# emsig/emg3d

Measured on AMD Instinct MI355X. Metric: Mcells*smoother-iters/s (fp64) per multigrid cycle, higher is better.
Workload: dtype c128 (complex fp64)

## Files before the change

emg3d_amd/_cycle.py:

```python
import os

import numpy as np
import torch

from emg3d_amd import _lib

__all__ = ['run_cycles', 'coarse_correction', 'coarse_schedule', 'smooth_level', 'stop_reason',
           'ConvergenceError', 'current_sc_dir', 'current_lr_dir']


class ConvergenceError(Exception):
    """Multigrid as preconditioner diverged or stagnated: aborts the Krylov solver."""


def current_sc_dir(sc_dir, grid):
    kept = tuple(n % 2 != 0 or n < 3 or sc_dir == axis + 1 for axis, n in enumerate(grid.shape_cells))
    codes = {(0, 0, 0): 0, (1, 0, 0): 1, (0, 1, 0): 2, (0, 0, 1): 3, (0, 1, 1): 4, (1, 0, 1): 5, (1, 1, 0): 6,
             (1, 1, 1): 6}
    return codes[tuple(int(k) for k in kept)]


_LR_AXES = {0: (), 1: (1,), 2: (2,), 3: (3,), 4: (2, 3), 5: (1, 3), 6: (1, 2), 7: (1, 2, 3)}
_LR_CODE = {axes: code for code, axes in _LR_AXES.items()}


def current_lr_dir(lr_dir, grid):
    axes = tuple(a for a in _LR_AXES[int(lr_dir)] if grid.shape_cells[a - 1] != 2)
    return _LR_CODE[axes]


def smooth_level(lv, nu, lr_dir, var):
    axes = _LR_AXES[current_lr_dir(lr_dir, lv.grid)]
# ... 28 lines not shown
            stack.pop()
            continue
        if level == depth:
            steps.append((SMOOTH, level, nu_coarse, "coarsest level", done, visits))
            frame[2] = done + 1
            continue
        if nu_pre > 0:
            steps.append((SMOOTH, level, nu_pre, "pre-smoothing", done, visits))
        steps.append((DOWN, level, 0))
        frame[3] = True
        steps.append((ENTER, level + 1, 0))
        stack.append([level + 1, _visits(cycle, cycmax, depth, level + 1, visits - done), 0, False])
    return steps


def _visits(cycle, cycmax, depth, level, budget):
    if level == depth:
        return 1
    if budget == 0 or cycle != 'F':
        return cycmax
    return budget


class CoarseCorrection:

    def __init__(self, first, first_level, var):
        self.var = var
        self.levels = {first_level: first}

    def run(self, steps):
        var = self.var
        loud = var.verb > 4
        trace = var.first_cycle and var.verb > 3
        sc_at = {}
        for step in steps:
            kind, level = step[0], step[1]
            lv = self.levels[level]
            if kind == SMOOTH:
                smooth_level(lv, step[2], var.lr_dir, var)
                if loud:
                    _log_smoothing(var, level, lv, step[3], step[4], step[5])
            elif kind == DOWN:
                sc_at[level] = current_sc_dir(var.sc_dir, lv.grid)
                lv.residual(store=True, norm=False)
                self.levels[level + 1] = lv.restrict_to(sc_at[level])
            elif kind == UP:
                lv.prolong_from(sc_at[level])
                if trace:
                    var.level_all.append(level)
            elif trace:
                var.level_all.append(level)


def _log_smoothing(var, level, lv, what, it=0, cycmax=None):
    n = lv.grid.shape_cells
    norm = lv.residual(store=False, norm=True)
    visits = var.cycmax if cycmax is None else cycmax
    var.cprint(f"     {it:2} {level} {visits} [{n[0]:3}, {n[1]:3}, {n[2]:3}]: {norm:.3e} {what}", 4)


USE_GRAPHS = os.environ.get('EMG3D_AMD_GRAPHS', '1') != '0'
GRAPH_AFTER = int(os.environ.get('EMG3D_AMD_GRAPH_AFTER', '2'))
CONCURRENT = 0


def coarse_correction(clv, var, budget, first_level=1, graphed=None, top=None):
    depth = int(var.clevel[var.sc_dir])
    steps = coarse_schedule(var.cycle, var.cycmax, depth, first_level, budget, var.nu_pre, var.nu_coarse,
                            var.nu_post)
    clv.work.factor_epoch += 1
    runner = CoarseCorrection(clv, first_level, var)
    if graphed is None:
        graphed = first_level == 1 and var.verb < 5 and USE_GRAPHS and CONCURRENT == 0
    if not graphed:
        runner.run(steps)
        return
    cache = clv.__dict__.setdefault('_graphs', {})
    key = (int(var.sc_dir), int(var.lr_dir), budget, var.cycle, var.nu_pre, var.nu_post, var.nu_coarse, depth,
           float(getattr(var, 'smoother_omega', 1.0)), _lib.options_fingerprint())
    entry = cache.get(key)
    if entry is None or entry['graph'] is None:
        if entry is None:
            stale = [k for k in cache if k[-1] != key[-1]]
            if stale:
                for k in stale:
                    del cache[k]
                root = top if top is not None else clv
                _purge_stale_graphs(root, key[-1])
                _drop_stale_point_factors(root)
            entry = cache[key] = {'work': None, 'graph': None, 'seen': 0}
        if entry['seen'] < GRAPH_AFTER:
            before = var.smoother_cell_sweeps
            runner.run(steps)
            entry['work'] = var.smoother_cell_sweeps - before
            entry['seen'] += 1
            return
        before = var.smoother_cell_sweeps
        torch.cuda.synchronize()
        graph = torch.cuda.CUDAGraph()
        with torch.cuda.graph(graph, capture_error_mode='thread_local'):
            runner.run(steps)
        entry['work'] = var.smoother_cell_sweeps - before
        var.smoother_cell_sweeps = before
        entry['graph'] = graph
    entry['graph'].replay()
    var.smoother_cell_sweeps += entry['work']


def _purge_stale_graphs(lv, fingerprint, seen=None):
    seen = set() if seen is None else seen
    if id(lv) in seen:
        return
    seen.add(id(lv))
    cache = lv.__dict__.get('_graphs')
    if cache:
        for k in [k for k in cache if k[-1] != fingerprint]:
            del cache[k]
    for link in lv.children.values():
        _purge_stale_graphs(link['level'], fingerprint, seen)


def _drop_stale_point_factors(lv, seen=None):
    seen = set() if seen is None else seen
    if id(lv) in seen:
        return
    seen.add(id(lv))
    now = ('point', _lib.lib().emg3d_get_option(b'point_tile_min'))
    for k in [k for k in lv._factors if isinstance(k, tuple) and k[0] == 'point' and k != now]:
        del lv._factors[k]
    for link in lv.children.values():
        _drop_stale_point_factors(link['level'], seen)


def stop_reason(var, l2_last, l2_stag, it):
# ... 173 lines not shown
```

emg3d_amd/_device.py:

```python
import ctypes

import numpy as np
import torch

from emg3d_amd import _lib, meshes
from emg3d_amd import core as _core

_vp = ctypes.c_void_p


def _stream():
    return _vp(torch.cuda.current_stream().cuda_stream)


def _ptr(t, offset_elems=0):
    return _vp(t.data_ptr() + offset_elems * t.element_size())


def coarsen_flags(sc_dir):
    return (sc_dir not in (1, 5, 6), sc_dir not in (2, 4, 6), sc_dir not in (3, 4, 5))


def interp_table(cnodes, nodes):
    i = np.searchsorted(cnodes, nodes) - 1
# ... 381 lines not shown
                ccc = (cgrid.cell_centers_x, cgrid.cell_centers_y, cgrid.cell_centers_z)[d]
                for w in _core.restrict_weights(nodes, cc, g.h[d], cnodes, ccc, cgrid.h[d]):
                    slots.append(len(fparts))
                    fparts.append(np.ascontiguousarray(w, dtype=np.float64))
            else:
                slots += [None, None, None]
        tabs = [interp_table(cn, n) for cn, n in ((cgrid.nodes_x, g.nodes_x),
                                                  (cgrid.nodes_y, g.nodes_y),
                                                  (cgrid.nodes_z, g.nodes_z))]
        pw_slots = []
        for t in tabs:
            pw_slots.append(len(fparts))
            fparts.append(t[1])
        foff = np.cumsum([0] + [a.size for a in fparts])
        fbuf = self.work.upload(np.concatenate(fparts))
        ioff = np.cumsum([0] + [t[0].size for t in tabs])
        ibuf = self.work.upload(np.concatenate([t[0] for t in tabs]))
        wptr = [(_ptr(fbuf, int(foff[i])) if i is not None else None) for i in slots]
        pwptr = [_ptr(fbuf, int(foff[i])) for i in pw_slots]
        ilptr = [_ptr(ibuf, int(ioff[d])) for d in range(3)]
        link = {'level': clevel, 'buffers': (fbuf, ibuf), 'wptr': wptr, 'ilptr': ilptr, 'pwptr': pwptr}
        self.children[sc_dir] = link
        return link

    def restrict_to(self, sc_dir):
        link = self.child(sc_dir)
        c = link['level']
        nx, ny, nz = self.grid.shape_cells
        _lib.check(_lib.lib().emg3d_dev_restrict_clear_batch(
            *c.parts(c.s), *c.parts(c.e), *self.parts(self.r), *link['wptr'], nx, ny, nz, sc_dir,
            self.is_complex, self.batch, self.grid.n_edges, c.grid.n_edges, _stream()), 'emg3d_dev_restrict')
        return c

    def prolong_from(self, sc_dir):
        link = self.children[sc_dir]
        c = link['level']
        nx, ny, nz = self.grid.shape_cells
        _lib.check(_lib.lib().emg3d_dev_prolong_batch(
            *self.parts(self.e), *c.parts(c.e), *link['ilptr'], *link['pwptr'], nx, ny, nz, sc_dir,
            self.is_complex, self.batch, self.grid.n_edges, c.grid.n_edges, _stream()),
            'emg3d_dev_prolong')
```

emg3d_amd/_lib.py:

```python
import ctypes
import os
import subprocess

_HERE = os.path.dirname(os.path.abspath(__file__))
CSRC = os.path.join(_HERE, 'csrc')
LIBDIR = os.path.join(_HERE, 'lib')
LIBPATH = os.path.join(LIBDIR, 'libemg3d_amd.so')
HEADER = os.path.join(os.path.dirname(_HERE), 'include', 'emg3d_amd.h')
SOURCES = [os.path.join(CSRC, f) for f in ('kernels.hip', 'stencil.h', 'launch.h', 'cplx.h', 'receivers.h', 'krylov.h',
                                            'adjoint.h', 'reciprocal.h', 'hessian.h', 'gram.h')] + [HEADER]

HIPCC_FLAGS = ['--offload-arch=gfx950', '-O3', '-std=c++17', '-fPIC', '-shared', '-ffp-contract=fast-honor-pragmas']


class Emg3dAmdError(RuntimeError):
    """A C-ABI call returned a non-zero status."""


def build(force=False, verbose=False):
    os.makedirs(LIBDIR, exist_ok=True)
    stale = (not os.path.exists(LIBPATH) or
             any(os.path.getmtime(s) > os.path.getmtime(LIBPATH) for s in SOURCES))
    if force or stale:
        hipcc = os.environ.get('HIPCC', 'hipcc')
# ... 21 lines not shown
    'emg3d_version': (_ci, []),
    'emg3d_last_error': (ctypes.c_char_p, []),
    'emg3d_device_count': (_ci, []),
    'emg3d_set_option': (_ci, [ctypes.c_char_p, _ci]),
    'emg3d_get_option': (_ci, [ctypes.c_char_p]),
    'emg3d_option_count': (_ci, []),
    'emg3d_option_name': (ctypes.c_char_p, [_ci]),
    'emg3d_options_generation': (_ci, []),
    'emg3d_line_kernel_name': (ctypes.c_char_p, [_ci] * 6),
    'emg3d_core_amat_x': (_ci, [_vp] * 13 + [_ci] * 4),
    'emg3d_core_gauss_seidel': (_ci, [_ci] + [_vp] * 13 + [_ci] * 5),
    'emg3d_core_restrict': (_ci, [_vp] * 15 + [_ci] * 5),
    'emg3d_core_blocks_to_amat': (_ci, [_vp] * 5 + [_ci] * 4),
    'emg3d_core_solve': (_ci, [_vp, _vp, _ci, _ci]),
    'emg3d_gs_scratch_bytes': (_sz, [_ci] * 5),
    'emg3d_line_fac_bytes': (_sz, [_ci] * 5),
    'emg3d_line_fac_bytes_lv': (_sz, [ctypes.POINTER(Level), _ci]),
    'emg3d_line_compact_used': (_ci, [ctypes.POINTER(Level), _ci]),
    'emg3d_point_compact_used': (_ci, [ctypes.POINTER(Level)]),
    'emg3d_line_lfac_bytes': (_sz, [_ci] * 4),
    'emg3d_dev_line_setup': (_ci, [ctypes.POINTER(Level), _ci, _vp, _vp, _vp]),
    'emg3d_point_fac_bytes': (_sz, [_ci] * 4),
    'emg3d_point_fac_bytes_lv': (_sz, [ctypes.POINTER(Level)]),
    'emg3d_dev_eta_is_imaginary': (_ci, [ctypes.POINTER(Level), ctypes.POINTER(_ci), _vp]),
    'emg3d_dev_point_setup': (_ci, [ctypes.POINTER(Level), _vp, _vp]),
    'emg3d_dev_gauss_seidel': (_ci, [ctypes.POINTER(Level), _ci, _ci, _vp, _vp, _vp, _sz, _vp]),
    'emg3d_residual_ws_len': (_sz, [_ci] * 3),
    'emg3d_dev_residual': (_ci, [ctypes.POINTER(Level), _vp, _vp, _vp, _vp, _sz, _vp, _vp]),
    'emg3d_dev_restrict': (_ci, [_vp] * 15 + [_ci] * 5 + [_vp]),
    'emg3d_dev_prolong': (_ci, [_vp] * 12 + [_ci] * 5 + [_vp]),
    'emg3d_dev_restrict_batch': (_ci, [_vp] * 15 + [_ci] * 6 + [_sz, _sz, _vp]),
    'emg3d_dev_restrict_clear_batch': (_ci, [_vp] * 18 + [_ci] * 6 + [_sz, _sz, _vp]),
    'emg3d_dev_prolong_batch': (_ci, [_vp] * 12 + [_ci] * 6 + [_sz, _sz, _vp]),
    'emg3d_dev_restrict_param': (_ci, [_vp, _vp] + [_ci] * 5 + [_vp]),
    'emg3d_dev_pec_zero': (_ci, [_vp] * 3 + [_ci] * 4 + [_vp]),
    'emg3d_krylov_ws_len': (_sz, []),
    'emg3d_dev_krylov_step': (_ci, [_sz, _ci, _vp, _ci, _vp, _vp, _vp, _ci, _vp, _vp, _vp, _ci, _vp, _vp, _vp, _sz, _vp]),
    'emg3d_dev_apply_operator': (_ci, [ctypes.POINTER(Level), _vp, _vp, _vp, _vp]),
    'emg3d_dev_zero': (_ci, [_vp, _sz, _vp]),
    'emg3d_dev_copy': (_ci, [_vp, _vp, _sz, _vp]),
    'emg3d_dev_gradient_accumulate': (_ci, [_ci] * 4 + [_vp] * 6 + [ctypes.c_double] * 2 + [_vp] * 5),
    'emg3d_dev_sensitivity_source': (_ci, [_ci] * 4 + [_vp] * 3 + [ctypes.c_double] * 2 + [_vp] * 7 + [_vp]),
    'emg3d_dev_edge_weights': (_ci, [_ci] * 3 + [_vp] * 7 + [_vp]),
    'emg3d_sensitivity_dots_ws_len': (_sz, [_ci, _ci, _sz]),
    'emg3d_dev_sensitivity_dots': (_ci, [_sz, _ci, _vp, _sz, _ci, _vp, _sz, _ci, _vp] + [ctypes.c_double] * 2 +
                                   [_vp, _vp, _sz, _vp]),
    'emg3d_dev_sensitivity_combine': (_ci, [_sz, _ci, _vp, _sz, _ci, _vp, _sz, _ci, _vp, _vp, _vp]),
    'emg3d_dev_edges_to_cells': (_ci, [_ci] * 4 + [_vp] * 3 + [ctypes.c_double] * 2 + [_vp] * 4 + [_vp]),
    'emg3d_dev_hessian_diagonal': (_ci, [_ci] * 4 + [_vp, _sz, _ci, _vp, _sz, _ci, _vp] + [_ci] * 3 + [ctypes.c_double] +
                                   [_vp, _vp, _sz, _vp]),
    'emg3d_data_gram_ws_len': (_sz, [_ci] * 6),
    'emg3d_dev_data_gram': (_ci, [_ci] * 4 + [_vp, _sz, _ci, _vp, _sz, _ci] + [ctypes.c_double] * 2 +
                            [_vp, _sz, _ci, _vp, _sz, _ci] + [ctypes.c_double] * 2 + [_ci] * 3 +
                            [_vp, _sz, _vp, _vp, _sz, _vp, _sz, _vp]),
    'emg3d_dev_source_field': (_ci, [_ci] * 4 + [_vp] * 7 + [_ci] + [ctypes.c_double] * 2 + [_vp] * 4),
    'emg3d_dev_volume_model': (_ci, [_ci] * 4 + [_vp] * 5 + [_ci] + [_vp] * 3 + [ctypes.c_double] * 4 + [_vp] * 5),
    'emg3d_dev_magnetic_field': (_ci, [_ci] * 4 + [_vp] * 7 + [ctypes.c_double] * 2 + [_vp] * 4),
    'emg3d_dev_spline_filter': (_ci, [_vp] + [_ci] * 4 + [_vp]),
    'emg3d_dev_spline_eval': (_ci, [_vp] + [_ci] * 4 + [_vp, _ci, _vp, _vp]),
    'emg3d_dev_linear_eval': (_ci, [_vp] + [_ci] * 4 + [_vp, _vp, _ci, _vp, _vp]),
    'emg3d_dev_volume_average': (_ci, [_vp] + [_ci] * 3 + [_vp] * 10 + [_ci] * 3 + [_vp, _ci, _vp]),
}

LEVEL_ETA_IMAG = 1
LEVEL_LINE_COMPACT = 2
LEVEL_POINT_COMPACT = 4
# ... 45 lines not shown
```

emg3d_amd/csrc/kernels.hip:

```cpp
#include <hip/hip_runtime.h>

#include <algorithm>
#include <climits>
#include <cstdio>
#include <cstdlib>
#include <cstring>
#include <string>
#include <type_traits>

#include "../../include/emg3d_amd.h"
#include "launch.h"

using emg::cplx;

namespace {

thread_local std::string g_err;

int fail(int code, const char *what)
{
    g_err = what;
    return code;
}

// ... 1339 lines not shown
        if (tid == 0) {
            const int bid = blockIdx.x + gridDim.x * (blockIdx.y + gridDim.y * blockIdx.z);
            partial[bid] = (wsum[0] + wsum[1]) + (wsum[2] + wsum[3]);
        }
    }
}

__global__ __launch_bounds__(256) void k_reduce_sum(const double *partial, int n, double *out)
{
    partial += (size_t)blockIdx.x * n;
    out += blockIdx.x;
    __shared__ double sm[256];
    double acc = 0.0;
    for (int i = threadIdx.x; i < n; i += 256) acc += partial[i];
    sm[threadIdx.x] = acc;
    __syncthreads();
    for (int s = 128; s > 0; s >>= 1) {
        if ((int)threadIdx.x < s) sm[threadIdx.x] += sm[threadIdx.x + s];
        __syncthreads();
    }
    if (threadIdx.x == 0) *out = sm[0];
}

template <class T> __global__ __launch_bounds__(256) void k_restrict(emg::Restrict<T> R)
{
    const int cix = blockIdx.x * blockDim.x + threadIdx.x;
    const int ciy = blockIdx.y * blockDim.y + threadIdx.y;
    const int b = blockIdx.z / R.cnzn, ciz = blockIdx.z - b * R.cnzn;
    if (cix >= R.cnxn || ciy >= R.cnyn) return;
    R.rx += b * R.fstride; R.ry += b * R.fstride; R.rz += b * R.fstride;
    R.crx += b * R.cstride; R.cry += b * R.cstride; R.crz += b * R.cstride;
    if (R.cex) { R.cex += b * R.cstride; R.cey += b * R.cstride; R.cez += b * R.cstride; }
    emg::restrict_node<T>(R, cix, ciy, ciz);
}

template <class T> __global__ __launch_bounds__(256) void k_prolong(emg::Prolong<T> P)
{
    const int ix = blockIdx.x * blockDim.x + threadIdx.x;
    const int iy = blockIdx.y * blockDim.y + threadIdx.y;
    const int b = blockIdx.z / (P.nz + 1), iz = blockIdx.z - b * (P.nz + 1);
    if (ix > P.nx || iy > P.ny) return;
    P.ex += b * P.fstride; P.ey += b * P.fstride; P.ez += b * P.fstride;
    P.cex += b * P.cstride; P.cey += b * P.cstride; P.cez += b * P.cstride;
    emg::prolong_cell<T>(P, ix, iy, iz);
}

template <class T>
__global__ __launch_bounds__(256) void k_restrict_param(T *out, const T *in, int nx, int ny, int cnx,
                                                        int cny, int fx, int fy, int fz)
{
    const int cix = blockIdx.x * blockDim.x + threadIdx.x;
    const int ciy = blockIdx.y * blockDim.y + threadIdx.y;
    const int ciz = blockIdx.z;
    if (cix >= cnx || ciy >= cny) return;
    emg::restrict_param_cell<T>(out, in, nx, ny, cnx, cny, fx, fy, fz, cix, ciy, ciz);
}

template <class T>
__global__ __launch_bounds__(256) void k_pec_zero(T *ex, T *ey, T *ez, int nx, int ny, int nz)
{
    const int ix = blockIdx.x * blockDim.x + threadIdx.x;
    const int iy = blockIdx.y * blockDim.y + threadIdx.y;
    const int iz = blockIdx.z;
    if (ix > nx || iy > ny) return;
    const bool bx = ix == 0 || ix == nx, by = iy == 0 || iy == ny, bz = iz == 0 || iz == nz;
    if (ix < nx && (by || bz)) ex[ix + nx * (iy + (ny + 1) * iz)] = emg::zero<T>();
// ... 369 lines not shown
template <class T>
int launch_restrict(void *crx, void *cry, void *crz, const void *rx, const void *ry, const void *rz,
                    const double *const w[9], int nx, int ny, int nz, int sc_dir, hipStream_t st, int batch = 1,
                    size_t fstride = 0, size_t cstride = 0, void *cex = nullptr, void *cey = nullptr, void *cez = nullptr)
{
    const ScDirs f = sc_flags(sc_dir);
    if ((f.cx && nx % 2) || (f.cy && ny % 2) || (f.cz && nz % 2))
        return fail(EMG3D_ERR_BADARG, "restrict: odd cell count in a coarsened direction");
    emg::Restrict<T> R = emg::make_restrict<T>(crx, cry, crz, rx, ry, rz, w, nx, ny, nz, sc_dir);
    R.batch = batch > 1 ? batch : 1; R.fstride = fstride; R.cstride = cstride;
    R.cex = (T *)cex; R.cey = (T *)cey; R.cez = (T *)cez;
    const emg::Dim3 g = emg::cell_grid(R.cnxn, R.cnyn, R.cnzn);
    hipLaunchKernelGGL(k_restrict<T>, dim3(g.x, g.y, g.z * R.batch), d3(emg::cell_block()), 0, st, R);
    HIP_TRY(hipGetLastError());
    return 0;
}

template <class T>
int launch_prolong(void *ex, void *ey, void *ez, const void *cex, const void *cey, const void *cez,
                   const int32_t *ilx, const int32_t *ily, const int32_t *ilz, const double *wx,
                   const double *wy, const double *wz, int nx, int ny, int nz, int sc_dir, hipStream_t st,
                   int batch = 1, size_t fstride = 0, size_t cstride = 0)
{
    emg::Prolong<T> P =
        emg::make_prolong<T>(ex, ey, ez, cex, cey, cez, ilx, ily, ilz, wx, wy, wz, nx, ny, nz, sc_dir);
    P.batch = batch > 1 ? batch : 1; P.fstride = fstride; P.cstride = cstride;
    const emg::Dim3 g = emg::cell_grid(nx + 1, ny + 1, nz + 1);
    hipLaunchKernelGGL(k_prolong<T>, dim3(g.x, g.y, g.z * P.batch), d3(emg::cell_block()), 0, st, P);
    HIP_TRY(hipGetLastError());
    return 0;
}

template <class T>
int launch_restrict_param(void *out, const void *in, int nx, int ny, int nz, int sc_dir, hipStream_t st)
{
    const ScDirs f = sc_flags(sc_dir);
    const int fx = f.cx ? 2 : 1, fy = f.cy ? 2 : 1, fz = f.cz ? 2 : 1;
    const int cnx = nx / fx, cny = ny / fy, cnz = nz / fz;
    const dim3 block = d3(emg::cell_block());
    const dim3 grid = d3(emg::cell_grid(cnx, cny, cnz));
    hipLaunchKernelGGL(k_restrict_param<T>, grid, block, 0, st, (T *)out, (const T *)in, nx, ny, cnx, cny, fx, fy, fz);
    HIP_TRY(hipGetLastError());
    return 0;
}


struct DevBuf {
    void *d = nullptr;
    size_t bytes = 0;
    ~DevBuf() { if (d) (void)hipFree(d); }
    hipError_t up(const void *h, size_t n)
    {
        bytes = n;
        hipError_t e = hipMalloc(&d, n ? n : 1);
        if (e != hipSuccess) return e;
        return n ? hipMemcpy(d, h, n, hipMemcpyHostToDevice) : hipSuccess;
    }
    hipError_t alloc(size_t n)
    {
        bytes = n;
        return hipMalloc(&d, n ? n : 1);
    }
    hipError_t down(void *h) const { return bytes ? hipMemcpy(h, d, bytes, hipMemcpyDeviceToHost) : hipSuccess; }
};

struct Sizes {
// ... 310 lines not shown
    const double *const w[9] = {wxl, wx0, wxr, wyl, wy0, wyr, wzl, wz0, wzr};
    return is_complex ? launch_restrict<cplx>(crx, cry, crz, rx, ry, rz, w, nx, ny, nz, sc_dir, (hipStream_t)stream, batch,
                                              fine_stride, coarse_stride)
                      : launch_restrict<double>(crx, cry, crz, rx, ry, rz, w, nx, ny, nz, sc_dir, (hipStream_t)stream,
                                                batch, fine_stride, coarse_stride);
}

int emg3d_dev_restrict_clear_batch(void *crx, void *cry, void *crz, void *cex, void *cey, void *cez, const void *rx,
                                   const void *ry, const void *rz, const double *wxl, const double *wx0,
                                   const double *wxr, const double *wyl, const double *wy0, const double *wyr,
                                   const double *wzl, const double *wz0, const double *wzr, int nx, int ny, int nz,
                                   int sc_dir, int is_complex, int batch, size_t fine_stride, size_t coarse_stride,
                                   void *stream)
{
    if (sc_dir < 0 || sc_dir > 6) return fail(EMG3D_ERR_BADARG, "restrict: sc_dir must be 0..6");
    if (!cex || !cey || !cez) return fail(EMG3D_ERR_BADARG, "restrict_clear: coarse field missing");
    const double *const w[9] = {wxl, wx0, wxr, wyl, wy0, wyr, wzl, wz0, wzr};
    return is_complex ? launch_restrict<cplx>(crx, cry, crz, rx, ry, rz, w, nx, ny, nz, sc_dir, (hipStream_t)stream, batch,
                                              fine_stride, coarse_stride, cex, cey, cez)
                      : launch_restrict<double>(crx, cry, crz, rx, ry, rz, w, nx, ny, nz, sc_dir, (hipStream_t)stream,
                                                batch, fine_stride, coarse_stride, cex, cey, cez);
}

int emg3d_dev_prolong_batch(void *ex, void *ey, void *ez, const void *cex, const void *cey, const void *cez,
                            const int32_t *ilx, const int32_t *ily, const int32_t *ilz, const double *wx,
                            const double *wy, const double *wz, int nx, int ny, int nz, int sc_dir, int is_complex,
                            int batch, size_t fine_stride, size_t coarse_stride, void *stream)
{
    if (sc_dir < 0 || sc_dir > 6) return fail(EMG3D_ERR_BADARG, "prolong: sc_dir must be 0..6");
    return is_complex ? launch_prolong<cplx>(ex, ey, ez, cex, cey, cez, ilx, ily, ilz, wx, wy, wz, nx, ny, nz, sc_dir,
                                             (hipStream_t)stream, batch, fine_stride, coarse_stride)
                      : launch_prolong<double>(ex, ey, ez, cex, cey, cez, ilx, ily, ilz, wx, wy, wz, nx, ny, nz, sc_dir,
                                               (hipStream_t)stream, batch, fine_stride, coarse_stride);
}

int emg3d_dev_restrict_param(void *out, const void *in, int nx, int ny, int nz, int sc_dir, int is_complex,
                             void *stream)
{
    if (sc_dir < 0 || sc_dir > 6) return fail(EMG3D_ERR_BADARG, "restrict_param: sc_dir must be 0..6");
    return is_complex ? launch_restrict_param<cplx>(out, in, nx, ny, nz, sc_dir, (hipStream_t)stream)
                      : launch_restrict_param<double>(out, in, nx, ny, nz, sc_dir, (hipStream_t)stream);
}

int emg3d_dev_pec_zero(void *ex, void *ey, void *ez, int nx, int ny, int nz, int is_complex, void *stream)
{
    const dim3 block = d3(emg::cell_block());
    const dim3 grid = d3(emg::cell_grid(nx + 1, ny + 1, nz + 1));
    if (is_complex)
        hipLaunchKernelGGL(k_pec_zero<cplx>, grid, block, 0, (hipStream_t)stream, (cplx *)ex, (cplx *)ey, (cplx *)ez, nx, ny, nz);
    else
        hipLaunchKernelGGL(k_pec_zero<double>, grid, block, 0, (hipStream_t)stream, (double *)ex, (double *)ey, (double *)ez, nx, ny, nz);
    HIP_TRY(hipGetLastError());
    return 0;
}


int emg3d_core_amat_x(void *rx, void *ry, void *rz, const void *ex, const void *ey, const void *ez,
                      const void *eta_x, const void *eta_y, const void *eta_z, const double *zeta,
                      const double *hx, const double *hy, const double *hz, int nx, int ny, int nz,
                      int is_complex)
{
    if (emg3d_device_count() < 1) return fail(EMG3D_ERR_NODEVICE, "no HIP device");
    const Sizes S(nx, ny, nz, is_complex);
    DevBuf drx, dry, drz, dex, dey, dez, dz, dhx, dhy, dhz;
    EtaUpload eta;
    HIP_TRY(drx.up(rx, S.nex * S.esz)); HIP_TRY(dry.up(ry, S.ney * S.esz)); HIP_TRY(drz.up(rz, S.nez * S.esz));
// ... 138 lines not shown
```

emg3d_amd/csrc/launch.h:

```cpp
#pragma once
#include "stencil.h"

namespace emg {

struct Dim3 { int x, y, z; };

inline int cdiv(int a, int b) { return (a + b - 1) / b; }
EMG_HD int fast_div(int a, int b) { return (int)(((float)a + 0.5f) / (float)b); }
inline int cnt_par(int n, int par) { return par ? n / 2 : (n - 1) / 2; }
EMG_HD int first_par(int par) { return par ? 1 : 2; }

inline int mirrored_colour(int iback, int cc)
{
    const int seq[4] = {0, 2, 3, 1};
    return seq[iback ? 3 - cc : cc];
}
inline int &point_order_ref() { static int order = 1; return order; }
inline int sweep_colour(int iback, int cc)
{
    return mirrored_colour(point_order_ref() == 0 ? iback : 0, cc);
}
inline int line_sweep_colour(int order, int it, int cc)
{
    if (order == 0) return mirrored_colour((it + 1) & 1, cc);
// ... 486 lines not shown
        for (int r = 0; r < 5; ++r) rhs[r] = zero<T>();
    }
    T *o = vec + ((size_t)k * (cntp * cntq) + lid) * 5;
#pragma unroll
    for (int r = 0; r < 5; ++r) o[r] = rhs[r];
}

template <class T, int DIR>
EMG_HD void line_scatter_thread(const Level<T> &L, int colour, int cntp, int cntq, int tp, int tq, int k,
                                const T *vec)
{
    int i1, i2, lid;
    if (!line_of_thread<DIR>(colour, cntp, cntq, tp, tq, i1, i2, lid)) return;
    const Axes<T, DIR> A(L);
    line_scatter<T, DIR>(A, k, i1, i2, vec + ((size_t)k * (cntp * cntq) + lid) * 5);
}

inline Dim3 linequad_block() { return Dim3{64, 1, 1}; }
inline Dim3 linequad_grid(const LineClass &c) { return Dim3{cdiv(c.lines * 4, 64), 1, 1}; }

inline Dim3 cell_block() { return Dim3{64, 4, 1}; }
inline Dim3 cell_grid(int n1, int n2, int n3) { return Dim3{cdiv(n1, 64), cdiv(n2, 4), n3}; }

struct ScDirs { int cx, cy, cz; };
inline ScDirs sc_flags(int sc_dir)
{
    ScDirs f;
    f.cx = !(sc_dir == 1 || sc_dir == 5 || sc_dir == 6);
    f.cy = !(sc_dir == 2 || sc_dir == 4 || sc_dir == 6);
    f.cz = !(sc_dir == 3 || sc_dir == 4 || sc_dir == 5);
    return f;
}

template <class T>
inline Restrict<T> make_restrict(void *crx, void *cry, void *crz, const void *rx, const void *ry,
                                 const void *rz, const double *const w[9], int nx, int ny, int nz, int sc_dir)
{
    const ScDirs f = sc_flags(sc_dir);
    Restrict<T> R;
    R.cx = f.cx; R.cy = f.cy; R.cz = f.cz;
    R.nxn = nx + 1; R.nyn = ny + 1; R.nzn = nz + 1;
    R.cnxn = (f.cx ? nx / 2 : nx) + 1; R.cnyn = (f.cy ? ny / 2 : ny) + 1; R.cnzn = (f.cz ? nz / 2 : nz) + 1;
    R.rx = (const T *)rx; R.ry = (const T *)ry; R.rz = (const T *)rz;
    R.crx = (T *)crx; R.cry = (T *)cry; R.crz = (T *)crz;
    for (int i = 0; i < 3; ++i) { R.wx[i] = w[i]; R.wy[i] = w[3 + i]; R.wz[i] = w[6 + i]; }
    return R;
}

template <class T>
inline Prolong<T> make_prolong(void *ex, void *ey, void *ez, const void *cex, const void *cey, const void *cez,
                               const int *ilx, const int *ily, const int *ilz, const double *wx,
                               const double *wy, const double *wz, int nx, int ny, int nz, int sc_dir)
{
    const ScDirs f = sc_flags(sc_dir);
    Prolong<T> P;
    P.cx = f.cx; P.cy = f.cy; P.cz = f.cz;
    P.nx = nx; P.ny = ny; P.nz = nz;
    P.cnx = f.cx ? nx / 2 : nx; P.cny = f.cy ? ny / 2 : ny; P.cnz = f.cz ? nz / 2 : nz;
    P.ex = (T *)ex; P.ey = (T *)ey; P.ez = (T *)ez;
    P.cex = (const T *)cex; P.cey = (const T *)cey; P.cez = (const T *)cez;
    P.ilx = ilx; P.ily = ily; P.ilz = ilz; P.wx = wx; P.wy = wy; P.wz = wz;
    return P;
}

}
```

emg3d_amd/csrc/stencil.h:

```cpp
#pragma once
#include "cplx.h"

namespace emg {

template <class T> struct Level {
    int nx, ny, nz;
    T *ex, *ey, *ez;
    const T *sx, *sy, *sz;
    const T *eta_x, *eta_y, *eta_z;
    const double *zeta;
    const double *ihx, *ihy, *ihz;
    int batch = 1;
    size_t bstride = 0;
    int flags = 0;
};
constexpr int LEVEL_ETA_IMAG = 1;
constexpr int LEVEL_LINE_COMPACT = 2;
constexpr int LEVEL_POINT_COMPACT = 4;
template <class T> EMG_HD Level<T> source_level(Level<T> L, int b)
{
    size_t o = (size_t)b * L.bstride;
#if defined(__HIP_DEVICE_COMPILE__)
    o = ((size_t)__builtin_amdgcn_readfirstlane((unsigned)(o >> 32)) << 32) | (size_t)__builtin_amdgcn_readfirstlane((unsigned)o);
#endif
// ... 256 lines not shown
    const bool inx = ix < nx, iny = iy < ny, inz = iz < nz;
    double acc = 0.0;

    if (inx && iny && inz) {
        T ox, oy, oz;
        residual_values<T, true>(L, ix, iy, iz, ox, oy, oz);
        acc = abs2(ox) + abs2(oy) + abs2(oz);
        if (rx) {
            rx[A.iex(ix, iy, iz)] = ox;
            ry[A.iey(ix, iy, iz)] = oy;
            rz[A.iez(ix, iy, iz)] = oz;
        }
    } else {
        if (inx) {
            const T v = L.sx[A.iex(ix, iy, iz)];
            acc += abs2(v);
            if (rx) rx[A.iex(ix, iy, iz)] = v;
        }
        if (iny) {
            const T v = L.sy[A.iey(ix, iy, iz)];
            acc += abs2(v);
            if (ry) ry[A.iey(ix, iy, iz)] = v;
        }
        if (inz) {
            const T v = L.sz[A.iez(ix, iy, iz)];
            acc += abs2(v);
            if (rz) rz[A.iez(ix, iy, iz)] = v;
        }
    }
    return acc;
}

template <class T>
EMG_HD double residual_column(const Level<T> &L, T *rx, T *ry, T *rz, int ix, int iy, int z0, int z1)
{
    const Axes<T, 0> A(L);
    double acc = 0.0;
    if (ix < L.nx && iy < L.ny) {
        ResIn<T> in;
        bool have = false;
        for (int iz = z0; iz < z1; ++iz) {
            if (iz < L.nz) {
                if (have) residual_load_roll<T>(L, ix, iy, iz, in);
                else residual_load<T>(L, ix, iy, iz, in);
                have = true;
                T ox, oy, oz;
                residual_compute<T, true>(L, in, ix, iy, iz, ox, oy, oz);
                acc += abs2(ox) + abs2(oy) + abs2(oz);
                if (rx) {
                    rx[A.iex(ix, iy, iz)] = ox;
                    ry[A.iey(ix, iy, iz)] = oy;
                    rz[A.iez(ix, iy, iz)] = oz;
                }
            } else {
                acc += residual_cell<T>(L, rx, ry, rz, ix, iy, iz);
            }
        }
    } else {
        for (int iz = z0; iz < z1; ++iz) acc += residual_cell<T>(L, rx, ry, rz, ix, iy, iz);
    }
    return acc;
}

EMG_HD constexpr bool pt_nz(int i, int j) { return !(i == 1 && j == 0); }

template <class T> EMG_HD void solve6(const T (&dg)[6], const double (&od)[6][6], T (&b)[6])
// ... 1089 lines not shown
            const int k = kb0 + (i + 1) * dk;
            T N[16];
            getN(kb0 + i * dk, N);
            wide_chain_step<T>(N, true, gh[k], v);
            for (int e = 0; e < 4; ++e) gh[k][e] = v[e];
        }
    }
    for (int j = 0; j < n0 - 2; ++j) {
        const WideBlock b = wide_block(j, mk);
        T Tk[15], x[5];
        getT(b.k, Tk);
        wide_x<T, 15>(Tk, c[b.k], gh[b.k], x);
        wide_block_scatter<T, DIR>(A, b.k, b.mir, i1, i2, x);
    }
    {
        const T xs[5] = {xq[0], xq[1], xq[2], xq[3], xq[4]};
        wide_block_scatter<T, DIR>(A, mk, 0, i1, i2, xs);
        A.E(0)[A.idx(0, mk + 1, i1, i2)] = xq[5];
    }
}

template <class T> struct Restrict {
    int cx, cy, cz;
    int nxn, nyn, nzn;
    int cnxn, cnyn, cnzn;
    const T *rx, *ry, *rz;
    T *crx, *cry, *crz;
    T *cex = nullptr, *cey = nullptr, *cez = nullptr;
    const double *wx[3], *wy[3], *wz[3];
    int batch = 1;
    size_t fstride = 0, cstride = 0;
};

template <class T> EMG_HD void restrict_node(const Restrict<T> &R, int cix, int ciy, int ciz)
{
    const int nx = R.nxn, ny = R.nyn, nz = R.nzn;
    const int cnx = R.cnxn, cny = R.cnyn;
    const int ix = R.cx ? 2 * cix : cix, iy = R.cy ? 2 * ciy : ciy, iz = R.cz ? 2 * ciz : ciz;
    int ixs[3], iys[3], izs[3];
    double wxs[3], wys[3], wzs[3];
    ixs[0] = ix; ixs[1] = ix > 0 ? ix - 1 : 0; ixs[2] = ix + 1 < nx - 1 ? ix + 1 : nx - 1;
    iys[0] = iy; iys[1] = iy > 0 ? iy - 1 : 0; iys[2] = iy + 1 < ny - 1 ? iy + 1 : ny - 1;
    izs[0] = iz; izs[1] = iz > 0 ? iz - 1 : 0; izs[2] = iz + 1 < nz - 1 ? iz + 1 : nz - 1;
    wxs[0] = R.cx ? R.wx[1][cix] : 1.0; wxs[1] = R.cx ? R.wx[0][cix] : 0.0; wxs[2] = R.cx ? R.wx[2][cix] : 0.0;
    wys[0] = R.cy ? R.wy[1][ciy] : 1.0; wys[1] = R.cy ? R.wy[0][ciy] : 0.0; wys[2] = R.cy ? R.wy[2][ciy] : 0.0;
    wzs[0] = R.cz ? R.wz[1][ciz] : 1.0; wzs[1] = R.cz ? R.wz[0][ciz] : 0.0; wzs[2] = R.cz ? R.wz[2][ciz] : 0.0;
    const int nxt = R.cx ? 3 : 1, nyt = R.cy ? 3 : 1, nzt = R.cz ? 3 : 1;

    if (cix < cnx - 1) {
        T acc = zero<T>();
        for (int a = 0; a < nyt; ++a) {
            T inner = zero<T>();
            for (int b = 0; b < nzt; ++b) {
                T v = R.rx[ix + (nx - 1) * (iys[a] + ny * izs[b])];
                if (R.cx) v += R.rx[ixs[2] + (nx - 1) * (iys[a] + ny * izs[b])];
                inner += wzs[b] * v;
            }
            acc += wys[a] * inner;
        }
        R.crx[cix + (cnx - 1) * (ciy + cny * ciz)] = acc;
        if (R.cex) R.cex[cix + (cnx - 1) * (ciy + cny * ciz)] = zero<T>();
    }
    if (ciy < cny - 1) {
        T acc = zero<T>();
        for (int a = 0; a < nxt; ++a) {
            T inner = zero<T>();
            for (int b = 0; b < nzt; ++b) {
                T v = R.ry[ixs[a] + nx * (iy + (ny - 1) * izs[b])];
                if (R.cy) v += R.ry[ixs[a] + nx * (iys[2] + (ny - 1) * izs[b])];
                inner += wzs[b] * v;
            }
            acc += wxs[a] * inner;
        }
        R.cry[cix + cnx * (ciy + (cny - 1) * ciz)] = acc;
        if (R.cey) R.cey[cix + cnx * (ciy + (cny - 1) * ciz)] = zero<T>();
    }
    if (ciz < R.cnzn - 1) {
        T acc = zero<T>();
        for (int a = 0; a < nxt; ++a) {
            T inner = zero<T>();
            for (int b = 0; b < nyt; ++b) {
                T v = R.rz[ixs[a] + nx * (iys[b] + ny * iz)];
                if (R.cz) v += R.rz[ixs[a] + nx * (iys[b] + ny * izs[2])];
                inner += wys[b] * v;
            }
            acc += wxs[a] * inner;
        }
        R.crz[cix + cnx * (ciy + cny * ciz)] = acc;
        if (R.cez) R.cez[cix + cnx * (ciy + cny * ciz)] = zero<T>();
    }
}

template <class T> struct Prolong {
    int cx, cy, cz;
    int nx, ny, nz;
    int cnx, cny, cnz;
    T *ex, *ey, *ez;
    const T *cex, *cey, *cez;
    const int *ilx, *ily, *ilz;
    const double *wx, *wy, *wz;
    int batch = 1;
    size_t fstride = 0, cstride = 0;
};

template <class T> EMG_HD void prolong_cell(const Prolong<T> &P, int ix, int iy, int iz)
{
    const int nx = P.nx, ny = P.ny, nz = P.nz, cnx = P.cnx, cny = P.cny;
    const bool ty = iy >= 1 && iy <= ny - 1, tz = iz >= 1 && iz <= nz - 1, tx = ix >= 1 && ix <= nx - 1;
    if (ix < nx && ty && tz) {
        const int cix = P.cx ? ix / 2 : ix;
        const int a = P.ily[iy], b = P.ilz[iz];
        const double wa = P.wy[iy], wb = P.wz[iz];
        const T *c = P.cex + cix;
        const T v = c[cnx * (a + (cny + 1) * b)] * ((1 - wa) * (1 - wb)) +
                    c[cnx * (a + (cny + 1) * (b + 1))] * ((1 - wa) * wb) +
                    c[cnx * (a + 1 + (cny + 1) * b)] * (wa * (1 - wb)) +
                    c[cnx * (a + 1 + (cny + 1) * (b + 1))] * (wa * wb);
        P.ex[ix + nx * (iy + (ny + 1) * iz)] += v;
    }
    if (iy < ny && tx && tz) {
        const int ciy = P.cy ? iy / 2 : iy;
        const int a = P.ilx[ix], b = P.ilz[iz];
        const double wa = P.wx[ix], wb = P.wz[iz];
// ... 87 lines not shown
```

include/emg3d_amd.h:

```cpp
#ifndef EMG3D_AMD_H
#define EMG3D_AMD_H

#include <stddef.h>
#include <stdint.h>

#ifdef __cplusplus
extern "C" {
#endif

#define EMG3D_AMD_VERSION 100

#define EMG3D_ERR_BADARG (-1)
#define EMG3D_ERR_NODEVICE (-2)
#define EMG3D_ERR_SCRATCH (-3)
#define EMG3D_ERR_INTERNAL (-4)

typedef struct emg3d_level {
    int32_t nx, ny, nz;
    int32_t is_complex;
    void *ex, *ey, *ez;
    const void *sx, *sy, *sz;
    const void *eta_x, *eta_y, *eta_z;
    const double *zeta;
    const double *ihx, *ihy, *ihz;
// ... 60 lines not shown
int emg3d_dev_residual(const emg3d_level *lv, void *rx, void *ry, void *rz, double *ws,
                       size_t ws_len, double *sumsq, void *stream);

int emg3d_dev_restrict(void *crx, void *cry, void *crz, const void *rx, const void *ry,
                       const void *rz, const double *wxl, const double *wx0, const double *wxr,
                       const double *wyl, const double *wy0, const double *wyr, const double *wzl,
                       const double *wz0, const double *wzr, int nx, int ny, int nz, int sc_dir,
                       int is_complex, void *stream);

int emg3d_dev_prolong(void *ex, void *ey, void *ez, const void *cex, const void *cey, const void *cez,
                      const int32_t *ilx, const int32_t *ily, const int32_t *ilz, const double *wx,
                      const double *wy, const double *wz, int nx, int ny, int nz, int sc_dir,
                      int is_complex, void *stream);

int emg3d_dev_restrict_batch(void *crx, void *cry, void *crz, const void *rx, const void *ry,
                             const void *rz, const double *wxl, const double *wx0, const double *wxr,
                             const double *wyl, const double *wy0, const double *wyr, const double *wzl,
                             const double *wz0, const double *wzr, int nx, int ny, int nz, int sc_dir,
                             int is_complex, int batch, size_t fine_stride, size_t coarse_stride,
                             void *stream);
int emg3d_dev_restrict_clear_batch(void *crx, void *cry, void *crz, void *cex, void *cey, void *cez,
                                   const void *rx, const void *ry, const void *rz, const double *wxl,
                                   const double *wx0, const double *wxr, const double *wyl,
                                   const double *wy0, const double *wyr, const double *wzl,
                                   const double *wz0, const double *wzr, int nx, int ny, int nz,
                                   int sc_dir, int is_complex, int batch, size_t fine_stride,
                                   size_t coarse_stride, void *stream);
int emg3d_dev_prolong_batch(void *ex, void *ey, void *ez, const void *cex, const void *cey,
                            const void *cez, const int32_t *ilx, const int32_t *ily, const int32_t *ilz,
                            const double *wx, const double *wy, const double *wz, int nx, int ny, int nz,
                            int sc_dir, int is_complex, int batch, size_t fine_stride,
                            size_t coarse_stride, void *stream);

int emg3d_dev_restrict_param(void *out, const void *in, int nx, int ny, int nz, int sc_dir,
                             int is_complex, void *stream);

int emg3d_dev_pec_zero(void *ex, void *ey, void *ez, int nx, int ny, int nz, int is_complex,
                       void *stream);

size_t emg3d_krylov_ws_len(void);
int emg3d_dev_krylov_step(size_t n, int is_complex, void *y, int nterms, const void *const *xs, const int *slots,
                          const double *scales, int ndots, const void *const *das, const void *const *dbs,
                          const int *dslots, int nprog, const int *prog, double *table, double *ws, size_t ws_len,
                          void *stream);
int emg3d_dev_apply_operator(const emg3d_level *lv, void *ox, void *oy, void *oz, void *stream);
int emg3d_dev_zero(void *p, size_t bytes, void *stream);
int emg3d_dev_copy(void *dst, const void *src, size_t bytes, void *stream);

int emg3d_dev_magnetic_field(int nx, int ny, int nz, int is_complex, const void *ex, const void *ey,
                             const void *ez, const double *zeta, const double *hx, const double *hy,
                             const double *hz, double smu0_re, double smu0_im, void *mx, void *my,
                             void *mz, void *stream);

int emg3d_dev_spline_filter(void *data, int n0, int n1, int n2, int is_complex, void *stream);
int emg3d_dev_spline_eval(const void *coef, int n0, int n1, int n2, int is_complex,
                          const double *coords, int npts, void *out, void *stream);
int emg3d_dev_linear_eval(const void *values, int n0, int n1, int n2, int is_complex,
                          const int32_t *idx, const double *w, int npts, void *out, void *stream);

int emg3d_dev_gradient_accumulate(int nx, int ny, int nz, int is_complex, const void *ex, const void *ey,
                                  const void *ez, const void *bx, const void *by, const void *bz,
                                  double smu0_re, double smu0_im, const double *volumes, double *gx,
                                  double *gy, double *gz, void *stream);

int emg3d_dev_sensitivity_source(int nx, int ny, int nz, int is_complex, const void *ex, const void *ey,
                                 const void *ez, double smu0_re, double smu0_im, const double *volumes,
// ... 52 lines not shown
```

Before: 3932.

## Fuse residual computation and restriction into one LDS-tiled kernel for small levels

Adds a kernel that computes the residual for a tile of fine cells into shared memory and then restricts it directly to coarse nodes. This skips writing the fine residual to global memory and launching a second kernel, but only on levels up to a fixed cell count. It is gated by an environment flag that defaults to on and is folded into the graph cache key. It also disables Python GC while a graph is being captured. Halo cells are recomputed per tile, and the fine residual is not stored on the fused path.

New measurement: 3903. No clear change (-0.8%).

```diff
diff --git a/emg3d_amd/_cycle.py b/emg3d_amd/_cycle.py
--- a/emg3d_amd/_cycle.py
+++ b/emg3d_amd/_cycle.py
@@ -1,3 +1,4 @@
+import gc
 import os
 
 import numpy as np
@@ -92,6 +93,7 @@
         var = self.var
         loud = var.verb > 4
         trace = var.first_cycle and var.verb > 3
+        fused = FUSED_TRANSFERS and not loud and not trace
         sc_at = {}
         for step in steps:
             kind, level = step[0], step[1]
@@ -102,6 +104,9 @@
                     _log_smoothing(var, level, lv, step[3], step[4], step[5])
             elif kind == DOWN:
                 sc_at[level] = current_sc_dir(var.sc_dir, lv.grid)
+                if fused:
+                    self.levels[level + 1] = lv.down_to(sc_at[level])
+                    continue
                 lv.residual(store=True, norm=False)
                 self.levels[level + 1] = lv.restrict_to(sc_at[level])
             elif kind == UP:
@@ -121,6 +126,7 @@
 
 USE_GRAPHS = os.environ.get('EMG3D_AMD_GRAPHS', '1') != '0'
 GRAPH_AFTER = int(os.environ.get('EMG3D_AMD_GRAPH_AFTER', '2'))
+FUSED_TRANSFERS = os.environ.get('EMG3D_AMD_FUSED_TRANSFERS', '1') != '0'
 CONCURRENT = 0
 
 
@@ -137,7 +143,7 @@
         return
     cache = clv.__dict__.setdefault('_graphs', {})
     key = (int(var.sc_dir), int(var.lr_dir), budget, var.cycle, var.nu_pre, var.nu_post, var.nu_coarse, depth,
-           float(getattr(var, 'smoother_omega', 1.0)), _lib.options_fingerprint())
+           float(getattr(var, 'smoother_omega', 1.0)), bool(FUSED_TRANSFERS), _lib.options_fingerprint())
     entry = cache.get(key)
     if entry is None or entry['graph'] is None:
         if entry is None:
@@ -158,8 +164,15 @@
         before = var.smoother_cell_sweeps
         torch.cuda.synchronize()
         graph = torch.cuda.CUDAGraph()
-        with torch.cuda.graph(graph, capture_error_mode='thread_local'):
-            runner.run(steps)
+        gc.collect()
+        gc_on = gc.isenabled()
+        gc.disable()
+        try:
+            with torch.cuda.graph(graph, capture_error_mode='thread_local'):
+                runner.run(steps)
+        finally:
+            if gc_on:
+                gc.enable()
         entry['work'] = var.smoother_cell_sweeps - before
         var.smoother_cell_sweeps = before
         entry['graph'] = graph
diff --git a/emg3d_amd/_device.py b/emg3d_amd/_device.py
--- a/emg3d_amd/_device.py
+++ b/emg3d_amd/_device.py
@@ -437,6 +437,27 @@
             self.is_complex, self.batch, self.grid.n_edges, c.grid.n_edges, _stream()), 'emg3d_dev_restrict')
         return c
 
+    def down_uses_fused(self, sc_dir):
+        if 'emg3d_residual_restrict_fused' not in _lib.SIGNATURES:
+            return False
+        nx, ny, nz = self.grid.shape_cells
+        return bool(_lib.lib().emg3d_residual_restrict_fused(nx, ny, nz, sc_dir, self.batch))
+
+    def residual_restrict_to(self, sc_dir, store=False):
+        link = self.child(sc_dir)
+        c = link['level']
+        r = self.parts(self.r) if store else (None, None, None)
+        _lib.check(_lib.lib().emg3d_dev_residual_restrict(
+            self._cref, *c.parts(c.s), *c.parts(c.e), *r, *link['wptr'], sc_dir, c.grid.n_edges, _stream()),
+            'emg3d_dev_residual_restrict')
+        return c
+
+    def down_to(self, sc_dir):
+        if self.down_uses_fused(sc_dir):
+            return self.residual_restrict_to(sc_dir)
+        self.residual(store=True, norm=False)
+        return self.restrict_to(sc_dir)
+
     def prolong_from(self, sc_dir):
         link = self.children[sc_dir]
         c = link['level']
diff --git a/emg3d_amd/_lib.py b/emg3d_amd/_lib.py
--- a/emg3d_amd/_lib.py
+++ b/emg3d_amd/_lib.py
@@ -77,6 +77,9 @@
     'emg3d_dev_restrict_batch': (_ci, [_vp] * 15 + [_ci] * 6 + [_sz, _sz, _vp]),
     'emg3d_dev_restrict_clear_batch': (_ci, [_vp] * 18 + [_ci] * 6 + [_sz, _sz, _vp]),
     'emg3d_dev_prolong_batch': (_ci, [_vp] * 12 + [_ci] * 6 + [_sz, _sz, _vp]),
+    'emg3d_residual_restrict_fused': (_ci, [_ci] * 5),
+    'emg3d_residual_restrict_tile': (_ci, [_ci] + [ctypes.POINTER(_ci)] * 3),
+    'emg3d_dev_residual_restrict': (_ci, [ctypes.POINTER(Level)] + [_vp] * 18 + [_ci, _sz, _vp]),
     'emg3d_dev_restrict_param': (_ci, [_vp, _vp] + [_ci] * 5 + [_vp]),
     'emg3d_dev_pec_zero': (_ci, [_vp] * 3 + [_ci] * 4 + [_vp]),
     'emg3d_krylov_ws_len': (_sz, []),
diff --git a/emg3d_amd/csrc/kernels.hip b/emg3d_amd/csrc/kernels.hip
--- a/emg3d_amd/csrc/kernels.hip
+++ b/emg3d_amd/csrc/kernels.hip
@@ -1395,6 +1395,50 @@
     R.crx += b * R.cstride; R.cry += b * R.cstride; R.crz += b * R.cstride;
     if (R.cex) { R.cex += b * R.cstride; R.cey += b * R.cstride; R.cez += b * R.cstride; }
     emg::restrict_node<T>(R, cix, ciy, ciz);
+}
+
+template <class T>
+__global__ __launch_bounds__(256) void k_residual_restrict(emg::Level<T> L0, emg::Restrict<T> R, T *rx, T *ry, T *rz, int ntz)
+{
+    __shared__ double2 rr_smem[3 * emg::RR_BOX_MAX];
+    T *const box = reinterpret_cast<T *>(rr_smem);
+    const int b = blockIdx.z / ntz, tz = blockIdx.z - b * ntz;
+    const emg::Level<T> L = emg::source_level(L0, b);
+    R.crx += b * R.cstride; R.cry += b * R.cstride; R.crz += b * R.cstride;
+    if (R.cex) { R.cex += b * R.cstride; R.cey += b * R.cstride; R.cez += b * R.cstride; }
+    if (rx) { rx += b * L0.bstride; ry += b * L0.bstride; rz += b * L0.bstride; }
+    const int tcx = R.cx ? emg::RR_TILE_C : emg::RR_TILE_K, tcy = R.cy ? emg::RR_TILE_C : emg::RR_TILE_K,
+              tcz = R.cz ? emg::RR_TILE_C : emg::RR_TILE_K;
+    const int c0x = blockIdx.x * tcx, c0y = blockIdx.y * tcy, c0z = tz * tcz;
+    const int c1x = min(c0x + tcx, R.cnxn), c1y = min(c0y + tcy, R.cnyn), c1z = min(c0z + tcz, R.cnzn);
+    const int ox = R.cx ? 2 * c0x : c0x, oy = R.cy ? 2 * c0y : c0y, oz = R.cz ? 2 * c0z : c0z;
+    const int x0 = R.cx ? max(ox - 1, 0) : ox, y0 = R.cy ? max(oy - 1, 0) : oy, z0 = R.cz ? max(oz - 1, 0) : oz;
+    const int x1 = R.cx ? min(2 * c1x - 1, R.nxn - 1) : c1x - 1, y1 = R.cy ? min(2 * c1y - 1, R.nyn - 1) : c1y - 1,
+              z1 = R.cz ? min(2 * c1z - 1, R.nzn - 1) : c1z - 1;
+    const int bx = x1 - x0 + 1, by = y1 - y0 + 1, bz = z1 - z0 + 1;
+    const int nbox = bx * by * bz;
+    T *const px = box, *const py = box + nbox, *const pz = box + 2 * nbox;
+    const emg::Axes<T, 0> A(L);
+    for (int i = threadIdx.x; i < nbox; i += 256) {
+        const int lx = i % bx, r = i / bx, ly = r % by, lz = r / by;
+        const int ix = x0 + lx, iy = y0 + ly, iz = z0 + lz;
+        T o[3];
+        bool has[3];
+        emg::residual_cell_values<T>(L, ix, iy, iz, o, has);
+        px[i] = o[0]; py[i] = o[1]; pz[i] = o[2];
+        if (rx && ix >= ox && iy >= oy && iz >= oz) {
+            if (has[0]) rx[A.iex(ix, iy, iz)] = o[0];
+            if (has[1]) ry[A.iey(ix, iy, iz)] = o[1];
+            if (has[2]) rz[A.iez(ix, iy, iz)] = o[2];
+        }
+    }
+    __syncthreads();
+    const emg::ResidualBox<T> src{px, py, pz, x0, y0, z0, bx, by};
+    const int ncx = c1x - c0x, ncy = c1y - c0y, nc = ncx * ncy * (c1z - c0z);
+    for (int i = threadIdx.x; i < nc; i += 256) {
+        const int lx = i % ncx, r = i / ncx, ly = r % ncy, lz = r / ncy;
+        emg::restrict_node_from<T>(R, src, c0x + lx, c0y + ly, c0z + lz);
+    }
 }
 
 template <class T> __global__ __launch_bounds__(256) void k_prolong(emg::Prolong<T> P)
@@ -1830,6 +1874,31 @@
 }
 
 template <class T>
+int launch_residual_restrict(const emg3d_level *lv, void *crx, void *cry, void *crz, void *cex, void *cey, void *cez,
+                             void *rx, void *ry, void *rz, const double *const w[9], int sc_dir, size_t cstride,
+                             hipStream_t st)
+{
+    emg::Level<T> L = to_level<T>(lv);
+    const ScDirs f = sc_flags(sc_dir);
+    if (L.nx < 2 || L.ny < 2 || L.nz < 2) return fail(EMG3D_ERR_BADARG, "residual_restrict: need >= 2 cells per direction");
+    if ((f.cx && L.nx % 2) || (f.cy && L.ny % 2) || (f.cz && L.nz % 2))
+        return fail(EMG3D_ERR_BADARG, "residual_restrict: odd cell count in a coarsened direction");
+    for (int d = 0; d < 3; ++d)
+        if ((d == 0 ? f.cx : d == 1 ? f.cy : f.cz) && (!w[3 * d] || !w[3 * d + 1] || !w[3 * d + 2]))
+            return fail(EMG3D_ERR_BADARG, "residual_restrict: weights of a coarsened direction missing");
+    if ((rx || ry || rz) && !(rx && ry && rz)) return fail(EMG3D_ERR_BADARG, "residual_restrict: rx, ry, rz all or none");
+    emg::Restrict<T> R = emg::make_restrict<T>(crx, cry, crz, nullptr, nullptr, nullptr, w, L.nx, L.ny, L.nz, sc_dir);
+    R.cstride = cstride;
+    R.cex = (T *)cex; R.cey = (T *)cey; R.cez = (T *)cez;
+    const emg::Dim3 t = emg::residual_restrict_tile(sc_dir);
+    const int ntz = cdiv(R.cnzn, t.z);
+    hipLaunchKernelGGL(k_residual_restrict<T>, dim3(cdiv(R.cnxn, t.x), cdiv(R.cnyn, t.y), ntz * L.batch), dim3(256), 0, st, L,
+                       R, (T *)rx, (T *)ry, (T *)rz, ntz);
+    HIP_TRY(hipGetLastError());
+    return 0;
+}
+
+template <class T>
 int launch_restrict_param(void *out, const void *in, int nx, int ny, int nz, int sc_dir, hipStream_t st)
 {
     const ScDirs f = sc_flags(sc_dir);
@@ -2206,6 +2275,34 @@
                                              (hipStream_t)stream, batch, fine_stride, coarse_stride)
                       : launch_prolong<double>(ex, ey, ez, cex, cey, cez, ilx, ily, ilz, wx, wy, wz, nx, ny, nz, sc_dir,
                                                (hipStream_t)stream, batch, fine_stride, coarse_stride);
+}
+
+int emg3d_residual_restrict_fused(int nx, int ny, int nz, int sc_dir, int batch)
+{
+    return emg::residual_restrict_fused(nx, ny, nz, sc_dir, batch) ? 1 : 0;
+}
+
+int emg3d_residual_restrict_tile(int sc_dir, int *tx, int *ty, int *tz)
+{
+    if (sc_dir < 0 || sc_dir > 6 || !tx || !ty || !tz) return fail(EMG3D_ERR_BADARG, "residual_restrict_tile: bad argument");
+    const emg::Dim3 t = emg::residual_restrict_tile(sc_dir);
+    *tx = t.x; *ty = t.y; *tz = t.z;
+    return 0;
+}
+
+int emg3d_dev_residual_restrict(const emg3d_level *lv, void *crx, void *cry, void *crz, void *cex, void *cey, void *cez,
+                                void *rx, void *ry, void *rz, const double *wxl, const double *wx0, const double *wxr,
+                                const double *wyl, const double *wy0, const double *wyr, const double *wzl,
+                                const double *wz0, const double *wzr, int sc_dir, size_t coarse_stride, void *stream)
+{
+    if (!lv || !crx || !cry || !crz) return fail(EMG3D_ERR_BADARG, "residual_restrict: bad argument");
+    if (sc_dir < 0 || sc_dir > 6) return fail(EMG3D_ERR_BADARG, "residual_restrict: sc_dir must be 0..6");
+    if ((cex || cey || cez) && !(cex && cey && cez)) return fail(EMG3D_ERR_BADARG, "residual_restrict: cex, cey, cez all or none");
+    const double *const w[9] = {wxl, wx0, wxr, wyl, wy0, wyr, wzl, wz0, wzr};
+    return lv->is_complex ? launch_residual_restrict<cplx>(lv, crx, cry, crz, cex, cey, cez, rx, ry, rz, w, sc_dir,
+                                                           coarse_stride, (hipStream_t)stream)
+                          : launch_residual_restrict<double>(lv, crx, cry, crz, cex, cey, cez, rx, ry, rz, w, sc_dir,
+                                                             coarse_stride, (hipStream_t)stream);
 }
 
 int emg3d_dev_restrict_param(void *out, const void *in, int nx, int ny, int nz, int sc_dir, int is_complex,
diff --git a/emg3d_amd/csrc/launch.h b/emg3d_amd/csrc/launch.h
--- a/emg3d_amd/csrc/launch.h
+++ b/emg3d_amd/csrc/launch.h
@@ -542,6 +542,25 @@
     return f;
 }
 
+constexpr int RR_TILE_C = 4, RR_TILE_K = 8;
+constexpr int RR_BOX_C = 2 * RR_TILE_C + 1;
+constexpr int RR_BOX_MAX = RR_BOX_C * RR_BOX_C * RR_BOX_C;
+static_assert(RR_TILE_K <= RR_BOX_C, "the LDS box is sized by the coarsened directions");
+inline Dim3 residual_restrict_tile(int sc_dir)
+{
+    const ScDirs f = sc_flags(sc_dir);
+    return Dim3{f.cx ? RR_TILE_C : RR_TILE_K, f.cy ? RR_TILE_C : RR_TILE_K, f.cz ? RR_TILE_C : RR_TILE_K};
+}
+constexpr size_t RR_FUSED_CELLS = 300000;
+inline bool residual_restrict_fused(int nx, int ny, int nz, int sc_dir, int batch)
+{
+    if (sc_dir < 0 || sc_dir > 6 || nx < 2 || ny < 2 || nz < 2) return false;
+    const ScDirs f = sc_flags(sc_dir);
+    if ((f.cx && nx % 2) || (f.cy && ny % 2) || (f.cz && nz % 2)) return false;
+    const size_t cells = (size_t)(nx + 1) * (ny + 1) * (nz + 1) * (batch > 1 ? batch : 1);
+    return cells <= RR_FUSED_CELLS;
+}
+
 template <class T>
 inline Restrict<T> make_restrict(void *crx, void *cry, void *crz, const void *rx, const void *ry,
                                  const void *rz, const double *const w[9], int nx, int ny, int nz, int sc_dir)
diff --git a/emg3d_amd/csrc/stencil.h b/emg3d_amd/csrc/stencil.h
--- a/emg3d_amd/csrc/stencil.h
+++ b/emg3d_amd/csrc/stencil.h
@@ -312,6 +312,22 @@
 }
 
 template <class T>
+EMG_HD void residual_cell_values(const Level<T> &L, int ix, int iy, int iz, T (&o)[3], bool (&has)[3])
+{
+    const Axes<T, 0> A(L);
+    const bool inx = ix < L.nx, iny = iy < L.ny, inz = iz < L.nz;
+    has[0] = inx; has[1] = iny; has[2] = inz;
+    if (inx && iny && inz) {
+        residual_values<T, true>(L, ix, iy, iz, o[0], o[1], o[2]);
+    } else {
+        o[0] = o[1] = o[2] = zero<T>();
+        if (inx) o[0] = L.sx[A.iex(ix, iy, iz)];
+        if (iny) o[1] = L.sy[A.iey(ix, iy, iz)];
+        if (inz) o[2] = L.sz[A.iez(ix, iy, iz)];
+    }
+}
+
+template <class T>
 EMG_HD double residual_column(const Level<T> &L, T *rx, T *ry, T *rz, int ix, int iy, int z0, int z1)
 {
     const Axes<T, 0> A(L);
@@ -1467,7 +1483,23 @@
     size_t fstride = 0, cstride = 0;
 };
 
-template <class T> EMG_HD void restrict_node(const Restrict<T> &R, int cix, int ciy, int ciz)
+template <class T> struct ResidualGlobal {
+    const T *rx, *ry, *rz;
+    int nx, ny;
+    EMG_HD T x(int i, int j, int k) const { return rx[i + (nx - 1) * (j + ny * k)]; }
+    EMG_HD T y(int i, int j, int k) const { return ry[i + nx * (j + (ny - 1) * k)]; }
+    EMG_HD T z(int i, int j, int k) const { return rz[i + nx * (j + ny * k)]; }
+};
+template <class T> struct ResidualBox {
+    const T *rx, *ry, *rz;
+    int x0, y0, z0, bx, by;
+    EMG_HD int at(int i, int j, int k) const { return (i - x0) + bx * ((j - y0) + by * (k - z0)); }
+    EMG_HD T x(int i, int j, int k) const { return rx[at(i, j, k)]; }
+    EMG_HD T y(int i, int j, int k) const { return ry[at(i, j, k)]; }
+    EMG_HD T z(int i, int j, int k) const { return rz[at(i, j, k)]; }
+};
+
+template <class T, class Src> EMG_HD void restrict_node_from(const Restrict<T> &R, const Src &src, int cix, int ciy, int ciz)
 {
     const int nx = R.nxn, ny = R.nyn, nz = R.nzn;
     const int cnx = R.cnxn, cny = R.cnyn;
@@ -1487,8 +1519,8 @@
         for (int a = 0; a < nyt; ++a) {
             T inner = zero<T>();
             for (int b = 0; b < nzt; ++b) {
-                T v = R.rx[ix + (nx - 1) * (iys[a] + ny * izs[b])];
-                if (R.cx) v += R.rx[ixs[2] + (nx - 1) * (iys[a] + ny * izs[b])];
+                T v = src.x(ix, iys[a], izs[b]);
+                if (R.cx) v += src.x(ixs[2], iys[a], izs[b]);
                 inner += wzs[b] * v;
             }
             acc += wys[a] * inner;
@@ -1501,8 +1533,8 @@
         for (int a = 0; a < nxt; ++a) {
             T inner = zero<T>();
             for (int b = 0; b < nzt; ++b) {
-                T v = R.ry[ixs[a] + nx * (iy + (ny - 1) * izs[b])];
-                if (R.cy) v += R.ry[ixs[a] + nx * (iys[2] + (ny - 1) * izs[b])];
+                T v = src.y(ixs[a], iy, izs[b]);
+                if (R.cy) v += src.y(ixs[a], iys[2], izs[b]);
                 inner += wzs[b] * v;
             }
             acc += wxs[a] * inner;
@@ -1515,8 +1547,8 @@
         for (int a = 0; a < nxt; ++a) {
             T inner = zero<T>();
             for (int b = 0; b < nyt; ++b) {
-                T v = R.rz[ixs[a] + nx * (iys[b] + ny * iz)];
-                if (R.cz) v += R.rz[ixs[a] + nx * (iys[b] + ny * izs[2])];
+                T v = src.z(ixs[a], iys[b], iz);
+                if (R.cz) v += src.z(ixs[a], iys[b], izs[2]);
                 inner += wys[b] * v;
             }
             acc += wxs[a] * inner;
@@ -1524,6 +1556,11 @@
         R.crz[cix + cnx * (ciy + cny * ciz)] = acc;
         if (R.cez) R.cez[cix + cnx * (ciy + cny * ciz)] = zero<T>();
     }
+}
+
+template <class T> EMG_HD void restrict_node(const Restrict<T> &R, int cix, int ciy, int ciz)
+{
+    restrict_node_from<T>(R, ResidualGlobal<T>{R.rx, R.ry, R.rz, R.nxn, R.nyn}, cix, ciy, ciz);
 }
 
 template <class T> struct Prolong {
diff --git a/include/emg3d_amd.h b/include/emg3d_amd.h
--- a/include/emg3d_amd.h
+++ b/include/emg3d_amd.h
@@ -116,6 +116,13 @@
                             int sc_dir, int is_complex, int batch, size_t fine_stride,
                             size_t coarse_stride, void *stream);
 
+int emg3d_residual_restrict_fused(int nx, int ny, int nz, int sc_dir, int batch);
+int emg3d_residual_restrict_tile(int sc_dir, int *tx, int *ty, int *tz);
+int emg3d_dev_residual_restrict(const emg3d_level *lv, void *crx, void *cry, void *crz, void *cex, void *cey,
+                                void *cez, void *rx, void *ry, void *rz, const double *wxl, const double *wx0,
+                                const double *wxr, const double *wyl, const double *wy0, const double *wyr,
+                                const double *wzl, const double *wz0, const double *wzr, int sc_dir,
+                                size_t coarse_stride, void *stream);
 int emg3d_dev_restrict_param(void *out, const void *in, int nx, int ny, int nz, int sc_dir,
                              int is_complex, void *stream);
 
```
